# nuggy875/NeRF_pytorch_paeng

Hardware: AMD Instinct MI355X
Metric: rays/sec (4096-ray batch, 64c+128f samples) + 800×800 frame render ms (higher is better)
Workload: dtype f32

## Files before the change

### nerf_pytorch_paeng_amd/csrc/mlp_train.hip

```cpp
#include <type_traits>
#include <vector>
#include "mlp_core.h"
#include "half_layout.h"

namespace minerf {

int stage_embed(const float*, const float*, int64_t, int, int, int, float*, hipStream_t);
int dgrad_f16s(const mi_nerf_net*, const void*, const float*, const float*, const float*, const unsigned*, const unsigned*, float*, float*, float*, int64_t, int,
               long long, long long, const unsigned*, hipStream_t);

struct DgradArgs {
    const char* stream;
    unsigned stream_bytes;
    const float* side;
    unsigned side_floats, o_dens_w, o_color_w;
    const float* d_raw;
    const unsigned* mask_h;
    const unsigned* mask_g;
    float* delta_h;
    float* delta_f;
    float* delta_d;
    long long P;
    long long n_valid;
    long long n_wtiles;
    int S, tpr;
    int D;
};

template <int NT>
__device__ __forceinline__ void acc_zero(f32x16 (&acc)[8]) {
#pragma unroll
    for (int t = 0; t < NT; ++t)
#pragma unroll
        for (int r = 0; r < 16; ++r) acc[t][r] = 0.0f;
}

template <int W>
__global__ __launch_bounds__(256) __attribute__((amdgpu_waves_per_eu(1, 1)))
void mlp_dgrad_kernel(const DgradArgs a) {
    constexpr int NT = W / 32;
    constexpr int HN = W / 2;
    constexpr int AL = 8;
    extern __shared__ __attribute__((aligned(16))) char smem[];
    float* side = (float*)(smem + RING_BYTES);
    const int tid = threadIdx.x;
    const int lane = tid & 63;
    const int wave = __builtin_amdgcn_readfirstlane(tid >> 6);
    const int col = lane & 31, hh = lane >> 5;

    for (unsigned i = tid * 4; i < a.side_floats; i += 256 * 4) *(f32x4*)(side + i) = *(const f32x4*)(a.side + i);

    const long long n_wg_tiles = (a.n_wtiles + 3) >> 2;
    if ((long long)blockIdx.x >= n_wg_tiles) return;

    WRing ring = ring_start(a.stream, a.stream_bytes, smem, wave, lane);

    f32x16 acc[8];
    f32x4 aq[8];
    float h[HN];
    ring_advance(ring);
#pragma unroll
    for (int t = 0; t < NT; ++t) aq[t] = ring_read(smem, ring, lane, t);

    const float* cw = side + a.o_color_w;
    const float* dw = side + a.o_dens_w;
    for (long long wgt = blockIdx.x; wgt < n_wg_tiles; wgt += gridDim.x) {
        long long wt = wgt * 4 + wave;
        const bool wave_active = wt < a.n_wtiles;
        if (!wave_active) wt = a.n_wtiles - 1;
        const long long ray = wt / a.tpr;
        const int sample = (int)(wt - ray * a.tpr) * 32 + col;
        long long idx = ray * a.S + (sample < a.S ? sample : a.S - 1);
        const bool valid = wave_active && sample < a.S && idx < a.n_valid;
        if (idx >= a.n_valid) idx = a.n_valid - 1;
        const f32x4 dr = *(const f32x4*)(a.d_raw + idx * 4);
        const u32x2 mgv = *(const u32x2*)(a.mask_g + (wt * 64 + lane) * 2);
        u32x4 mhv = *(const u32x4*)(a.mask_h + (((long long)(a.D - 1) * a.n_wtiles + wt) * 64 + lane) * 4);

        float h2[HN / 2];
        {
            const unsigned mg[2] = {mgv[0], mgv[1]};
#pragma unroll
            for (int q = 0; q < HN / 8; ++q) {
                const f32x4 w0 = *(const f32x4*)(cw + 8 * q + 4 * hh);
                const f32x4 w1 = *(const f32x4*)(cw + W / 2 + 8 * q + 4 * hh);
                const f32x4 w2 = *(const f32x4*)(cw + W + 8 * q + 4 * hh);
#pragma unroll
                for (int e = 0; e < 4; ++e) {
                    float v = dr[0] * w0[e];
                    v = __builtin_fmaf(dr[1], w1[e], v);
                    v = __builtin_fmaf(dr[2], w2[e], v);
                    h2[4 * q + e] = mask_apply(v, q, e, mg);
                }
            }
        }
        acc_zero<NT>(acc);
        {
            float* row = a.delta_d + idx * (W / 2) + 4 * hh;
            auto hook = [&](int kq, int t) __attribute__((always_inline)) { if (t == NT - 1) store_chunk(h2, kq, row); };
            gemm_part<NT, HN / 2, NT, AL>(acc, h2, aq, smem, ring, lane, hook);
        }
        acc_to_b<NT, false>(acc, h);
        acc_zero<NT>(acc);
        {
            float* row = a.delta_f + idx * W + 4 * hh;
            auto hook = [&](int kq, int t) __attribute__((always_inline)) { if (t == NT - 1) store_chunk(h, kq, row); };
            gemm_part<NT, HN, NT, AL>(acc, h, aq, smem, ring, lane, hook);
        }
        {
            const unsigned mw[4] = {mhv[0], mhv[1], mhv[2], mhv[3]};
            if (a.D > 1) mhv = *(const u32x4*)(a.mask_h + (((long long)(a.D - 2) * a.n_wtiles + wt) * 64 + lane) * 4);
            const float ds = dr[3];
#pragma unroll
            for (int q = 0; q < 4 * NT; ++q) {
                const f32x4 wv = *(const f32x4*)(dw + 8 * q + 4 * hh);
#pragma unroll
                for (int e = 0; e < 4; ++e)
                    h[4 * q + e] = mask_apply(__builtin_fmaf(wv[e], ds, acc[q >> 2][4 * (q & 3) + e]), q, e, mw);
            }
        }
#pragma unroll 1
        for (int l = a.D - 1; l > 0; --l) {
            float* row = a.delta_h + ((long long)l * a.P + idx) * W + 4 * hh;
            acc_zero<NT>(acc);
            auto hook = [&](int kq, int t) __attribute__((always_inline)) { if (t == NT - 1) store_chunk(h, kq, row); };
            gemm_part<NT, HN, NT, AL>(acc, h, aq, smem, ring, lane, hook);
            const unsigned mw[4] = {mhv[0], mhv[1], mhv[2], mhv[3]};
            if (l > 1) mhv = *(const u32x4*)(a.mask_h + (((long long)(l - 2) * a.n_wtiles + wt) * 64 + lane) * 4);
#pragma unroll
            for (int q = 0; q < 4 * NT; ++q)
#pragma unroll
                for (int e = 0; e < 4; ++e) h[4 * q + e] = mask_apply(acc[q >> 2][4 * (q & 3) + e], q, e, mw);
        }
        store_rows<NT>(h, a.delta_h + idx * W + 4 * hh, valid);
    }
    asm volatile("s_waitcnt vmcnt(0)" ::: "memory");
    __syncthreads();
}

constexpr int WG_MAXB = 12;
struct WgradArgs {
    const float* dlt[WG_MAXB]; const float* x[WG_MAXB];
    int ldd[WG_MAXB], ldx[WG_MAXB], M[WG_MAXB], N[WG_MAXB];
    int want_bias[WG_MAXB];
    long long P;
    float* partial;
    float* bpartial;
    int slices;
};
struct ReduceBatch {
    float* out[WG_MAXB]; float* bias[WG_MAXB];
    int ldo[WG_MAXB], M[WG_MAXB], N[WG_MAXB];
};

typedef unsigned u32x4 __attribute__((ext_vector_type(4)));
__device__ __forceinline__ __amdgpu_buffer_rsrc_t wg_rsrc(const float* base, long long row0, long long ld, long long P, int rows) {
    long long left = P - row0;
    left = left < 0 ? 0 : (left > rows ? rows : left);
    return __builtin_amdgcn_make_buffer_rsrc((void*)(base + row0 * ld), 0, (int)(left * ld * 4), 0x00020000);
}
__global__ __launch_bounds__(256) __attribute__((amdgpu_waves_per_eu(1, 1)))
void wgrad_big_kernel(const WgradArgs a) {
    constexpr int U = 6;
    __shared__ f32x4 bshare[2][64];
    const int lane = threadIdx.x & 63;
    const int wave = __builtin_amdgcn_readfirstlane(threadIdx.x >> 6);
    const int i = lane & 31, kh = lane >> 5;
    const unsigned nwg = gridDim.x * gridDim.y, v = blockIdx.y * gridDim.x + blockIdx.x;
    const unsigned xcd = v & 7, slot = v >> 3;
    const unsigned full = nwg >> 3, rem = nwg & 7;
    const unsigned flat = xcd * full + (xcd < rem ? xcd : rem) + slot;
    const int b = (int)(flat / gridDim.x);
    const unsigned slice = flat - (unsigned)b * gridDim.x;
    const int wm = wave >> 1, wn = wave & 1;
    const int m0 = wm * 128, n0 = wn * 128;
    const bool aok = m0 + 4 * i < a.M[b], bok = n0 + 4 * i < a.N[b];
    const float* abase = a.dlt[b];
    const float* bbase = a.x[b];
    const long long ldd = a.ldd[b], ldx = a.ldx[b];
    const bool want_bias = a.want_bias[b] != 0;

    f32x16 acc[4][4];
#pragma unroll
    for (int tm = 0; tm < 4; ++tm)
#pragma unroll
        for (int tn = 0; tn < 4; ++tn)
#pragma unroll
            for (int r = 0; r < 16; ++r) acc[tm][tn][r] = 0.0f;
    f32x4 bsum = {0.f, 0.f, 0.f, 0.f};

    const long long slices = gridDim.x;
    unsigned voa[U], vob[U];
#pragma unroll
    for (int u = 0; u < U; ++u) {
        voa[u] = aok ? (unsigned)(((2 * u + kh) * ldd + m0 + 4 * i) * 4) : 0x80000000u;
        vob[u] = bok ? (unsigned)(((2 * u + kh) * ldx + n0 + 4 * i) * 4) : 0x80000000u;
    }
    long long req_group = slice;
    f32x4 ca[U], cb[U], na[U], nb[U], fa[U], fb[U];
    __amdgpu_buffer_rsrc_t ra, rb;
    auto open_group = [&]() __attribute__((always_inline)) {
        const long long row0 = req_group * (2 * U);
        ra = wg_rsrc(abase, row0, ldd, a.P, 2 * U);
        rb = wg_rsrc(bbase, row0, ldx, a.P, 2 * U);
        req_group += slices;
    };
    auto request = [&](int u, f32x4& A, f32x4& B) __attribute__((always_inline)) {
        A = __builtin_bit_cast(f32x4, __builtin_amdgcn_raw_buffer_load_b128(ra, voa[u], 0, 0));
        B = __builtin_bit_cast(f32x4, __builtin_amdgcn_raw_buffer_load_b128(rb, vob[u], 0, 0));
    };
    open_group();
#pragma unroll
    for (int u = 0; u < U; ++u) request(u, ca[u], cb[u]);
    open_group();
#pragma unroll
    for (int u = 0; u < U; ++u) request(u, na[u], nb[u]);
    auto step = [&](auto PAR, f32x4 (&A)[U], f32x4 (&B)[U], f32x4 (&FA)[U], f32x4 (&FB)[U]) __attribute__((always_inline)) {
        constexpr int par = decltype(PAR)::value;
        open_group();
#pragma unroll
        for (int u = 0; u < U; ++u) {
#pragma unroll
            for (int tm = 0; tm < 4; ++tm)
#pragma unroll
                for (int tn = 0; tn < 4; ++tn)
                    acc[tm][tn] = __builtin_amdgcn_mfma_f32_32x32x2f32(A[u][tm], B[u][tn], acc[tm][tn], 0, 0, 0);
            if ((u & 1) == par) bsum += A[u];
            request(u, FA[u], FB[u]);
            __builtin_amdgcn_sched_barrier(0);
        }
    };
    const long long all_groups = (a.P + 2 * U - 1) / (2 * U);
    const long long n_groups = (all_groups + slices - 1) / slices;
    auto loop = [&](auto PAR) __attribute__((always_inline)) {
        long long g = 0;
        do {
            step(PAR, ca, cb, fa, fb);
            step(PAR, na, nb, ca, cb);
            step(PAR, fa, fb, na, nb);
            g += 3;
        } while (g < n_groups);
    };
    if (!want_bias) loop(std::integral_constant<int, -1>{});
    else if (wn == 0) loop(std::integral_constant<int, 0>{});
    else loop(std::integral_constant<int, 1>{});
    const int lane_o = (int)__builtin_amdgcn_mbcnt_hi(~0u, __builtin_amdgcn_mbcnt_lo(~0u, 0u));
    const int i_o = lane_o & 31, kh_o = lane_o >> 5;
    float* out = a.partial + ((size_t)b * a.slices + slice) * (256 * 256);
#pragma unroll
    for (int tm = 0; tm < 4; ++tm)
#pragma unroll
        for (int r = 0; r < 16; ++r) {
            const int m = m0 + 4 * ((r & 3) + 8 * (r >> 2) + 4 * kh_o) + tm;
            f32x4 v;
#pragma unroll
            for (int tn = 0; tn < 4; ++tn) asm volatile("v_accvgpr_read_b32 %0, %1" : "=v"(v[tn]) : "a"(acc[tm][tn][r]));
            *(f32x4*)(out + (size_t)m * 256 + n0 + 4 * i_o) = v;
        }
    if (want_bias) {
        if (wn == 1) bshare[wm][lane_o] = bsum;
        __syncthreads();
        if (wn == 0) {
            bsum += bshare[wm][lane_o];
            f32x4 sv;
#pragma unroll
            for (int e = 0; e < 4; ++e) sv[e] = bsum[e] + __shfl_xor(bsum[e], 32, 64);
            if (kh_o == 0) *(f32x4*)(a.bpartial + ((size_t)b * a.slices + slice) * 256 + m0 + 4 * i_o) = sv;
        }
    }
}

typedef _Float16 f16x8 __attribute__((ext_vector_type(8)));
__global__ __launch_bounds__(256) void absmax_kernel(const float* __restrict__ x, long long n, unsigned* __restrict__ out_bits) {
    float m = 0.0f;
    const long long n4 = ((uintptr_t)x & 15) == 0 ? n >> 2 : 0;
    for (long long i = (long long)blockIdx.x * 256 + threadIdx.x; i < n4; i += (long long)gridDim.x * 256) {
        const f32x4 v = ((const f32x4*)x)[i];
        m = __builtin_fmaxf(__builtin_fmaxf(m, __builtin_fmaxf(__builtin_fabsf(v[0]), __builtin_fabsf(v[1]))), __builtin_fmaxf(__builtin_fabsf(v[2]), __builtin_fabsf(v[3])));
    }
    for (long long i = 4 * n4 + (long long)blockIdx.x * 256 + threadIdx.x; i < n; i += (long long)gridDim.x * 256) m = __builtin_fmaxf(m, __builtin_fabsf(x[i]));
#pragma unroll
    for (int o = 32; o > 0; o >>= 1) m = __builtin_fmaxf(m, __shfl_xor(m, o, 64));
    if ((threadIdx.x & 63) == 0 && m == m) atomicMax(out_bits, __float_as_uint(m));
}
static void launch_absmax(const float* x, long long n, unsigned* out_bits, hipStream_t st) {
    long long blocks = (n / 4 + 255) / 256;
    blocks = blocks < 1 ? 1 : (blocks > 4096 ? 4096 : blocks);
    hipLaunchKernelGGL(absmax_kernel, dim3((unsigned)blocks), dim3(256), 0, st, x, n, out_bits);
}
template <bool S>
__device__ __forceinline__ void split_pair(float v0, float v1, float s, unsigned& hi, unsigned& lo) {
    if constexpr (S) { v0 *= s; v1 *= s; }
    asm("v_cvt_pk_f16_f32 %0, %1, %2" : "=v"(hi) : "v"(v0), "v"(v1));
    asm("v_fma_mixlo_f16 %0, %1, -1.0, %2 op_sel_hi:[1,0,0]\n\tv_fma_mixhi_f16 %0, %1, -1.0, %3 op_sel:[1,0,0] op_sel_hi:[1,0,0]"
        : "=&v"(lo) : "v"(hi), "v"(v0), "v"(v1));
}
template <int BIAS>
__device__ __forceinline__ void wgrad_f16s_body(const WgradArgs& a, const unsigned* absmax_bits, f32x4 (*bshare)[64]) {
    const int lane = threadIdx.x & 63;
    const int wave = __builtin_amdgcn_readfirstlane(threadIdx.x >> 6);
    const int i = lane & 31, kh = lane >> 5;
    const unsigned nwg = gridDim.x * gridDim.y, v = blockIdx.y * gridDim.x + blockIdx.x;
    const unsigned xcd = v & 7, slot = v >> 3;
    const unsigned full = nwg >> 3, rem = nwg & 7;
    const unsigned flat = xcd * full + (xcd < rem ? xcd : rem) + slot;
    const int b = (int)(flat / gridDim.x);
    const unsigned slice = flat - (unsigned)b * gridDim.x;
    const int wm = wave >> 1, wn = wave & 1;
    const int m0 = wm * 128, n0 = wn * 128;
    const bool aok = m0 + 4 * i < a.M[b], bok = n0 + 4 * i < a.N[b];
    const float* abase = a.dlt[b];
    const float* bbase = a.x[b];
    const long long ldd = a.ldd[b], ldx = a.ldx[b];
    const unsigned mb = __builtin_amdgcn_readfirstlane((int)*absmax_bits);
    int e = (int)((mb >> 23) & 255u) - 127;
    if (mb == 0u || e < -100) e = -100;
    if (e > 100) e = 100;
    const float sc = __uint_as_float((unsigned)(127 + 7 - e) << 23), inv_sc = __uint_as_float((unsigned)(127 - 7 + e) << 23);

    f32x16 acc[4][4];
#pragma unroll
    for (int tm = 0; tm < 4; ++tm)
#pragma unroll
        for (int tn = 0; tn < 4; ++tn)
#pragma unroll
            for (int r = 0; r < 16; ++r) acc[tm][tn][r] = 0.0f;
    f32x4 bsum = {0.f, 0.f, 0.f, 0.f};

    constexpr int GROUP = 32;
    const long long slices = gridDim.x;
    unsigned voa[4], vob[4];
#pragma unroll
    for (int r = 0; r < 4; ++r) {
        voa[r] = aok ? (unsigned)(((8 * kh + r) * ldd + m0 + 4 * i) * 4) : 0x80000000u;
        vob[r] = bok ? (unsigned)(((8 * kh + r) * ldx + n0 + 4 * i) * 4) : 0x80000000u;
    }
    long long req_group = slice;
    struct Unit { f32x4 A[4], B[4]; };
    auto request = [&](int q, Unit& u) __attribute__((always_inline)) {
        const long long row0 = req_group * GROUP + 16 * (q >> 1) + 4 * (q & 1);
        const __amdgpu_buffer_rsrc_t ra = wg_rsrc(abase, row0, ldd, a.P, 12), rb = wg_rsrc(bbase, row0, ldx, a.P, 12);
#pragma unroll
        for (int r = 0; r < 4; ++r) {
            u.A[r] = __builtin_bit_cast(f32x4, __builtin_amdgcn_raw_buffer_load_b128(ra, voa[r], 0, 0));
            u.B[r] = __builtin_bit_cast(f32x4, __builtin_amdgcn_raw_buffer_load_b128(rb, vob[r], 0, 0));
        }
    };
    auto open_group = [&]() __attribute__((always_inline)) { req_group += slices; };
    unsigned ahi[4][4], alo[4][4], bhi[4][4], blo[4][4];
    auto convert = [&](int h, const Unit& u) __attribute__((always_inline)) {
#pragma unroll
        for (int t = 0; t < 4; ++t)
#pragma unroll
            for (int pr = 0; pr < 2; ++pr) {
                split_pair<true>(u.A[2 * pr][t], u.A[2 * pr + 1][t], sc, ahi[t][2 * h + pr], alo[t][2 * h + pr]);
                split_pair<false>(u.B[2 * pr][t], u.B[2 * pr + 1][t], 1.0f, bhi[t][2 * h + pr], blo[t][2 * h + pr]);
            }
        if constexpr (BIAS) {
#pragma unroll
            for (int r = 0; r < 4; ++r) bsum += u.A[r];
        }
    };
    auto mfmas = [&]() __attribute__((always_inline)) {
        f16x8 AH[4], AL[4], BH[4], BL[4];
#pragma unroll
        for (int t = 0; t < 4; ++t) {
            u32x4 w;
            w[0] = ahi[t][0]; w[1] = ahi[t][1]; w[2] = ahi[t][2]; w[3] = ahi[t][3]; AH[t] = __builtin_bit_cast(f16x8, w);
            w[0] = alo[t][0]; w[1] = alo[t][1]; w[2] = alo[t][2]; w[3] = alo[t][3]; AL[t] = __builtin_bit_cast(f16x8, w);
            w[0] = bhi[t][0]; w[1] = bhi[t][1]; w[2] = bhi[t][2]; w[3] = bhi[t][3]; BH[t] = __builtin_bit_cast(f16x8, w);
            w[0] = blo[t][0]; w[1] = blo[t][1]; w[2] = blo[t][2]; w[3] = blo[t][3]; BL[t] = __builtin_bit_cast(f16x8, w);
        }
#pragma unroll
        for (int tm = 0; tm < 4; ++tm)
#pragma unroll
            for (int tn = 0; tn < 4; ++tn) {
                acc[tm][tn] = __builtin_amdgcn_mfma_f32_32x32x16_f16(AH[tm], BH[tn], acc[tm][tn], 0, 0, 0);
                acc[tm][tn] = __builtin_amdgcn_mfma_f32_32x32x16_f16(AH[tm], BL[tn], acc[tm][tn], 0, 0, 0);
                acc[tm][tn] = __builtin_amdgcn_mfma_f32_32x32x16_f16(AL[tm], BH[tn], acc[tm][tn], 0, 0, 0);
            }
    };
    Unit u0, u1, u2, u3;
    request(0, u0); request(1, u1); request(2, u2); request(3, u3);
    const long long all_groups = (a.P + GROUP - 1) / GROUP;
    const long long n_groups = (all_groups + slices - 1) / slices;
    for (long long g = 0; g < n_groups; ++g) {
        open_group();
        convert(0, u0); request(0, u0);
        convert(1, u1); request(1, u1);
        mfmas();
        convert(0, u2); request(2, u2);
        convert(1, u3); request(3, u3);
        mfmas();
    }
    const int lane_o = (int)__builtin_amdgcn_mbcnt_hi(~0u, __builtin_amdgcn_mbcnt_lo(~0u, 0u));
    const int i_o = lane_o & 31, kh_o = lane_o >> 5;
    float* out = a.partial + ((size_t)b * a.slices + slice) * (256 * 256);
#pragma unroll
    for (int tm = 0; tm < 4; ++tm)
#pragma unroll
        for (int r = 0; r < 16; ++r) {
            const int m = m0 + 4 * ((r & 3) + 8 * (r >> 2) + 4 * kh_o) + tm;
            f32x4 vv;
#pragma unroll
            for (int tn = 0; tn < 4; ++tn) { float t; asm volatile("v_accvgpr_read_b32 %0, %1" : "=v"(t) : "a"(acc[tm][tn][r])); vv[tn] = t * inv_sc; }
            *(f32x4*)(out + (size_t)m * 256 + n0 + 4 * i_o) = vv;
        }
    if (a.want_bias[b] != 0) {
        if constexpr (BIAS) {
            f32x4 sv;
#pragma unroll
            for (int c = 0; c < 4; ++c) sv[c] = bsum[c] + __shfl_xor(bsum[c], 32, 64);
            if (kh_o == 0) *(f32x4*)(a.bpartial + ((size_t)b * a.slices + slice) * 256 + m0 + 4 * i_o) = sv;
        }
    }
    (void)bshare;
}
__global__ __launch_bounds__(256) __attribute__((amdgpu_waves_per_eu(1, 1)))
void wgrad_f16s_kernel(const WgradArgs a, const unsigned* absmax_bits) {
    asm volatile("s_setreg_imm32_b32 hwreg(HW_REG_MODE, 23, 1), 1");
    const int wave = __builtin_amdgcn_readfirstlane(threadIdx.x >> 6);
    if ((wave & 1) == 0) wgrad_f16s_body<1>(a, absmax_bits, nullptr);
    else wgrad_f16s_body<0>(a, absmax_bits, nullptr);
}

struct NarrowArgs {
    const float* wide; int ldw; int Mw;
    const float* nar;  int ldn; int Nn;
    long long P;
    int pps;
    float* partial;
    float* wsum;
    float* nsum;
};

template <int WQ, int NN, bool BW, bool BN>
__global__ __launch_bounds__(256) __attribute__((amdgpu_waves_per_eu(1, (WQ * NN == 4) ? 1 : 2)))
void wgrad_narrow_kernel(const NarrowArgs a) {
    constexpr int U = (WQ == 2) ? 4 : 6;
    const int lane = threadIdx.x & 63;
    const int wave = __builtin_amdgcn_readfirstlane(threadIdx.x >> 6);
    const int i = lane & 31, kh = lane >> 5;
    const long long slice = (long long)blockIdx.x * 4 + wave;
    const long long pb = slice * a.pps;
    const long long pe = pb >= a.P ? pb : ((pb + a.pps < a.P) ? pb + a.pps : a.P);
    const long long ldw = a.ldw, ldn = a.ldn;

    unsigned vow[U][WQ], von[U][NN];
#pragma unroll
    for (int u = 0; u < U; ++u) {
#pragma unroll
        for (int q = 0; q < WQ; ++q) vow[u][q] = (128 * q + 4 * i < a.Mw) ? (unsigned)(((2 * u + kh) * ldw + 128 * q + 4 * i) * 4) : 0x80000000u;
#pragma unroll
        for (int q = 0; q < NN; ++q) von[u][q] = (32 * q + i < a.Nn) ? (unsigned)(((2 * u + kh) * ldn + 32 * q + i) * 4) : 0x80000000u;
    }

    f32x16 acc[4 * WQ][NN];
#pragma unroll
    for (int tm = 0; tm < 4 * WQ; ++tm)
#pragma unroll
        for (int tn = 0; tn < NN; ++tn)
#pragma unroll
            for (int r = 0; r < 16; ++r) acc[tm][tn][r] = 0.0f;
    f32x4 wsum[WQ];
    float nsum[NN];
#pragma unroll
    for (int q = 0; q < WQ; ++q) wsum[q] = f32x4{0.f, 0.f, 0.f, 0.f};
#pragma unroll
    for (int q = 0; q < NN; ++q) nsum[q] = 0.0f;

    struct Set { f32x4 w[U][WQ]; float n[U][NN]; };
    Set c, nx, f;
    long long req_row = pb;
    __amdgpu_buffer_rsrc_t rw, rn;
    auto open_group = [&]() __attribute__((always_inline)) {
        rw = wg_rsrc(a.wide, req_row, ldw, pe, 2 * U);
        rn = wg_rsrc(a.nar, req_row, ldn, pe, 2 * U);
        req_row += 2 * U;
    };
    auto request = [&](Set& S, int u) __attribute__((always_inline)) {
#pragma unroll
        for (int q = 0; q < WQ; ++q) S.w[u][q] = __builtin_bit_cast(f32x4, __builtin_amdgcn_raw_buffer_load_b128(rw, vow[u][q], 0, 0));
#pragma unroll
        for (int q = 0; q < NN; ++q) S.n[u][q] = __builtin_bit_cast(float, __builtin_amdgcn_raw_buffer_load_b32(rn, von[u][q], 0, 0));
    };
    open_group();
#pragma unroll
    for (int u = 0; u < U; ++u) request(c, u);
    open_group();
#pragma unroll
    for (int u = 0; u < U; ++u) request(nx, u);
    auto step = [&](Set& A, Set& F) __attribute__((always_inline)) {
        open_group();
#pragma unroll
        for (int u = 0; u < U; ++u) {
#pragma unroll
            for (int tm = 0; tm < 4 * WQ; ++tm)
#pragma unroll
                for (int tn = 0; tn < NN; ++tn)
                    acc[tm][tn] = __builtin_amdgcn_mfma_f32_32x32x2f32(A.w[u][tm >> 2][tm & 3], A.n[u][tn], acc[tm][tn], 0, 0, 0);
            if (BW) {
#pragma unroll
                for (int q = 0; q < WQ; ++q) wsum[q] += A.w[u][q];
            }
            if (BN) {
#pragma unroll
                for (int q = 0; q < NN; ++q) nsum[q] += A.n[u][q];
            }
            request(F, u);
            __builtin_amdgcn_sched_barrier(0);
        }
    };
    const long long n_groups = (pe - pb + 2 * U - 1) / (2 * U);
    for (long long g = 0; g < n_groups; g += 3) {
        step(c, f);
        step(nx, c);
        step(f, nx);
    }
    constexpr int Wp = 128 * WQ, Np = 32 * NN;
    __shared__ float red[3][16][64];
    const __amdgpu_buffer_rsrc_t rout = __builtin_amdgcn_make_buffer_rsrc((void*)(a.partial + (size_t)blockIdx.x * Wp * Np), 0, Wp * Np * 4, 0x00020000);
    const unsigned vout = (unsigned)((16 * kh * Np + i) * 4);
#pragma unroll
    for (int tm = 0; tm < 4 * WQ; ++tm)
#pragma unroll
        for (int tn = 0; tn < NN; ++tn) {
            float t[16];
#pragma unroll
            for (int r = 0; r < 16; ++r) asm volatile("v_accvgpr_read_b32 %0, %1" : "=v"(t[r]) : "a"(acc[tm][tn][r]));
            if (wave > 0) {
#pragma unroll
                for (int r = 0; r < 16; ++r) red[wave - 1][r][lane] = t[r];
            }
            __syncthreads();
            if (wave == 0) {
#pragma unroll
                for (int r = 0; r < 16; ++r) {
                    const float v = ((t[r] + red[0][r][lane]) + red[1][r][lane]) + red[2][r][lane];
                    const int w0 = 128 * (tm >> 2) + 4 * ((r & 3) + 8 * (r >> 2)) + (tm & 3);
                    __builtin_amdgcn_raw_buffer_store_b32(__builtin_bit_cast(unsigned, v), rout, vout, (w0 * Np + 32 * tn) * 4, 0);
                }
            }
            __syncthreads();
        }
    float* sums = &red[0][0][0];
#pragma unroll
    for (int q = 0; q < WQ; ++q)
#pragma unroll
        for (int e = 0; e < 4; ++e) {
            const float v = wsum[q][e] + __shfl_xor(wsum[q][e], 32, 64);
            if (kh == 0) sums[wave * (Wp + Np) + 128 * q + 4 * i + e] = v;
        }
#pragma unroll
    for (int q = 0; q < NN; ++q) {
        const float v = nsum[q] + __shfl_xor(nsum[q], 32, 64);
        if (kh == 0) sums[wave * (Wp + Np) + Wp + 32 * q + i] = v;
    }
    __syncthreads();
    for (int c = threadIdx.x; c < Wp + Np; c += 256) {
        const float v = ((sums[c] + sums[(Wp + Np) + c]) + sums[2 * (Wp + Np) + c]) + sums[3 * (Wp + Np) + c];
        if (c < Wp) { if (a.wsum) a.wsum[(size_t)blockIdx.x * Wp + c] = v; }
        else if (a.nsum) a.nsum[(size_t)blockIdx.x * Np + (c - Wp)] = v;
    }
}

__global__ __launch_bounds__(256) void reduce_partial_kernel(const float* __restrict__ partial, const float* __restrict__ bpartial,
                                                              int slices, int Mp, int Np, int M, int N, float* __restrict__ out, int ldo,
                                                              float* __restrict__ bias, int bias_pitch, int transposed) {
    __shared__ float red[4][64];
    const int g = threadIdx.x >> 6, o = threadIdx.x & 63;
    const int idx = blockIdx.x * 64 + o;
    const int total = M * N + (bias ? M : 0);
    float acc = 0.0f;
    if (idx < M * N) {
        const int m = idx / N, n = idx - m * N;
        const float* p = partial + (transposed ? (size_t)n * Np + m : (size_t)m * Np + n);
        const size_t stride = (size_t)Mp * Np;
        float s[8] = {0.f, 0.f, 0.f, 0.f, 0.f, 0.f, 0.f, 0.f};
        int sl = g;
        for (; sl + 28 < slices; sl += 32) {
#pragma unroll
            for (int k = 0; k < 8; ++k) s[k] += p[(size_t)(sl + 4 * k) * stride];
        }
        for (; sl < slices; sl += 4) s[0] += p[(size_t)sl * stride];
        acc = ((s[0] + s[1]) + (s[2] + s[3])) + ((s[4] + s[5]) + (s[6] + s[7]));
    } else if (idx < total) {
        const int m = idx - M * N;
        for (int sl = g; sl < slices; sl += 4) acc += bpartial[(size_t)sl * bias_pitch + m];
    }
    red[g][o] = acc;
    __syncthreads();
    if (g == 0 && idx < total) {
        const float v = ((red[0][o] + red[1][o]) + red[2][o]) + red[3][o];
        if (idx < M * N) { const int m = idx / N, n = idx - m * N; out[(size_t)m * ldo + n] = v; }
        else bias[idx - M * N] = v;
    }
}

__global__ __launch_bounds__(256) void reduce_batch_kernel(const float* __restrict__ partial, const float* __restrict__ bpartial, int slices,
                                                            const ReduceBatch rb) {
    __shared__ float red[4][64];
    const int b = blockIdx.y;
    const int M = rb.M[b], N = rb.N[b];
    const int g = threadIdx.x >> 6, o = threadIdx.x & 63;
    const int idx = blockIdx.x * 64 + o;
    const int total = M * N + (rb.bias[b] ? M : 0);
    float acc = 0.0f;
    if (idx < M * N) {
        const int m = idx / N, n = idx - m * N;
        const float* p = partial + (size_t)b * slices * 65536 + (size_t)m * 256 + n;
        float s[8] = {0.f, 0.f, 0.f, 0.f, 0.f, 0.f, 0.f, 0.f};
        int sl = g;
        for (; sl + 28 < slices; sl += 32) {
#pragma unroll
            for (int k = 0; k < 8; ++k) s[k] += p[(size_t)(sl + 4 * k) * 65536];
        }
        for (; sl < slices; sl += 4) s[0] += p[(size_t)sl * 65536];
        acc = ((s[0] + s[1]) + (s[2] + s[3])) + ((s[4] + s[5]) + (s[6] + s[7]));
    } else if (idx < total) {
        const int m = idx - M * N;
        for (int sl = g; sl < slices; sl += 4) acc += bpartial[((size_t)b * slices + sl) * 256 + m];
    }
    red[g][o] = acc;
    __syncthreads();
    if (g == 0 && idx < total) {
        const float v = ((red[0][o] + red[1][o]) + red[2][o]) + red[3][o];
        if (idx < M * N) { const int m = idx / N, n = idx - m * N; rb.out[b][(size_t)m * rb.ldo[b] + n] = v; }
        else rb.bias[b][idx - M * N] = v;
    }
}

__global__ __launch_bounds__(256) void pack_apply_kernel(const int32_t* __restrict__ map, const float* __restrict__ flat, long long n,
                                                          float* __restrict__ blob) {
    const long long i = (long long)blockIdx.x * 256 + threadIdx.x;
    if (i >= n) return;
    const int32_t m = map[i];
    blob[i] = m > 0 ? flat[m - 1] : 0.0f;
}


static inline size_t al256(size_t v) { return (v + 255) & ~(size_t)255; }
constexpr size_t WGRAD_OVERRUN_PAD = 128 * 1024;

constexpr size_t WGRAD_PARTIAL_FLOATS = (size_t)256 * 256 * 256 + (size_t)256 * 256;

int train_layout(const mi_nerf_net* net, int64_t n_rays, int S, mi_nerf_train_layout* L) {
    MN_CHECK_ARG(net && L, "NULL net/layout");
    MN_CHECK_ARG(native_width(net->W), "the training kernels exist for W = 128 and 256 (got %d; inference pads narrower networks)", net->W);
    MN_CHECK_ARG(net->D >= 2 && net->D <= 16, "unsupported depth D=%d", net->D);
    MN_CHECK_ARG(n_rays >= 0 && S >= 1, "bad sizes n_rays=%lld S=%d", (long long)n_rays, S);
    const size_t p = (size_t)n_rays * S, W = (size_t)net->W, D = (size_t)net->D;
    const size_t n_wtiles = (size_t)n_rays * ((S + 31) / 32);
    const size_t in_all = (size_t)(3 + 6 * net->L_x) + (size_t)(3 + 6 * net->L_d);
    size_t off = 0;
    L->stash_h = off; off += al256(D * p * W * 4);
    L->stash_f = off; off += al256(p * W * 4);
    L->stash_g = off; off += al256(p * (W / 2) * 4) + WGRAD_OVERRUN_PAD;
    L->mask_h = off;  off += al256(D * n_wtiles * 64 * 16);
    L->mask_g = off;  off += al256(n_wtiles * 64 * 8);
    L->stash_bytes = off;
    off = 0;
    L->delta_h = off; off += al256(D * p * W * 4);
    L->delta_f = off; off += al256(p * W * 4);
    L->delta_d = off; off += al256(p * (W / 2) * 4) + WGRAD_OVERRUN_PAD;
    L->emb = off;     off += al256(p * in_all * 4);
    L->partial = off; off += al256(WGRAD_PARTIAL_FLOATS * 4);
    off += 256;
    L->work_bytes = off;
    return MI_NERF_OK;
}

struct WideProduct { const float* dlt; int ldd, M; const float* x; int ldx, N; float* out; int ldo; float* bias; };

static int run_wgrad_batch(const WideProduct* pr, int n, long long P, float* partial, hipStream_t st, const unsigned* absmax = nullptr) {
    MN_CHECK_ARG(n >= 1 && n <= WG_MAXB, "%d wide products in one batch (at most WG_MAXB)", n);
    WgradArgs a{};
    ReduceBatch rb{};
    int max_total = 0;
    for (int b = 0; b < n; ++b) {
        const WideProduct& q = pr[b];
        MN_CHECK_ARG(q.M <= 256 && q.N <= 256 && q.M % 4 == 0 && q.N % 4 == 0 && q.ldd % 4 == 0 && q.ldx % 4 == 0 &&
                     ((uintptr_t)q.dlt & 15) == 0 && ((uintptr_t)q.x & 15) == 0,
                     "wgrad operands must be at most 256 wide, 16-byte aligned, with pitches of 4 floats");
        a.dlt[b] = q.dlt; a.x[b] = q.x; a.ldd[b] = q.ldd; a.ldx[b] = q.ldx; a.M[b] = q.M; a.N[b] = q.N; a.want_bias[b] = q.bias != nullptr;
        rb.out[b] = q.out; rb.bias[b] = q.bias; rb.ldo[b] = q.ldo; rb.M[b] = q.M; rb.N[b] = q.N;
        const int total = q.M * q.N + (q.bias ? q.M : 0);
        if (total > max_total) max_total = total;
    }
    int slices = device_cus() / n;
    const long long all_groups = (P + 11) / 12;
    if (slices > all_groups) slices = (int)all_groups;
    if (slices < 1) slices = 1;
    MN_CHECK_ARG((size_t)n * slices * (65536 + 256) <= WGRAD_PARTIAL_FLOATS, "internal: wgrad partial buffer too small");
    a.P = P; a.slices = slices;
    a.partial = partial;
    a.bpartial = partial + (size_t)n * slices * 65536;
    if (absmax) hipLaunchKernelGGL(wgrad_f16s_kernel, dim3(slices, n), dim3(256), 0, st, a, absmax);
    else hipLaunchKernelGGL(wgrad_big_kernel, dim3(slices, n), dim3(256), 0, st, a);
    MN_LAUNCH_CHECK("wgrad_big_kernel");
    hipLaunchKernelGGL(reduce_batch_kernel, dim3((max_total + 63) / 64, n), dim3(256), 0, st, (const float*)partial, (const float*)a.bpartial,
                       slices, rb);
    MN_LAUNCH_CHECK("reduce_batch_kernel");
    return MI_NERF_OK;
}

static int run_wgrad(const float* dlt, int ldd, int M, const float* x, int ldx, int N, long long P, float* out, int ldo, float* bias,
                     float* partial, hipStream_t st) {
    if (M > 64 && N > 64) {
        const WideProduct q{dlt, ldd, M, x, ldx, N, out, ldo, bias};
        return run_wgrad_batch(&q, 1, P, partial, st);
    }
    const bool delta_is_wide = M >= N;
    NarrowArgs a{};
    a.wide = delta_is_wide ? dlt : x; a.ldw = delta_is_wide ? ldd : ldx; a.Mw = delta_is_wide ? M : N;
    a.nar = delta_is_wide ? x : dlt;  a.ldn = delta_is_wide ? ldx : ldd; a.Nn = delta_is_wide ? N : M;
    a.P = P;
    MN_CHECK_ARG(a.Mw <= 256 && a.Nn <= 64 && a.Mw % 4 == 0 && a.ldw % 4 == 0 && ((uintptr_t)a.wide & 15) == 0,
                 "unsupported narrow wgrad shape %d x %d", M, N);
    const int WQ = a.Mw > 128 ? 2 : 1, NN = a.Nn > 32 ? 2 : 1;
    const int Wp = 128 * WQ, Np = 32 * NN;
    const size_t per_slice = (size_t)Wp * Np + Wp + Np;
    long long wslices = 4LL * device_cus();
    long long pps = (P + wslices - 1) / wslices;
    pps = (pps + 23) / 24 * 24;
    wslices = (P + pps - 1) / pps;
    const long long slices = (wslices + 3) / 4;
    MN_CHECK_ARG((size_t)slices * per_slice <= WGRAD_PARTIAL_FLOATS, "internal: wgrad partial buffer too small");
    a.pps = (int)pps;
    a.partial = partial;
    float* wsum = partial + (size_t)slices * Wp * Np;
    float* nsum = wsum + (size_t)slices * Wp;
    a.wsum = (bias && delta_is_wide) ? wsum : nullptr;
    a.nsum = (bias && !delta_is_wide) ? nsum : nullptr;
    const dim3 grid((unsigned)slices);
    const bool bw = a.wsum != nullptr, bn = a.nsum != nullptr;
#define MN_NARROW(WQ_, NN_)                                                                                                   \
    do {                                                                                                                      \
        if (bw) hipLaunchKernelGGL((wgrad_narrow_kernel<WQ_, NN_, true, false>), grid, dim3(256), 0, st, a);                  \
        else if (bn) hipLaunchKernelGGL((wgrad_narrow_kernel<WQ_, NN_, false, true>), grid, dim3(256), 0, st, a);             \
        else hipLaunchKernelGGL((wgrad_narrow_kernel<WQ_, NN_, false, false>), grid, dim3(256), 0, st, a);                    \
    } while (0)
    if (WQ == 2 && NN == 2) MN_NARROW(2, 2);
    else if (WQ == 2) MN_NARROW(2, 1);
    else if (NN == 2) MN_NARROW(1, 2);
    else MN_NARROW(1, 1);
#undef MN_NARROW
    MN_LAUNCH_CHECK("wgrad_narrow_kernel");
    const int total = M * N + (bias ? M : 0);
    hipLaunchKernelGGL(reduce_partial_kernel, dim3((total + 63) / 64), dim3(256), 0, st, (const float*)partial,
                       (const float*)(delta_is_wide ? wsum : nsum), (int)slices, Wp, Np, M, N, out, ldo, bias, delta_is_wide ? Wp : Np,
                       delta_is_wide ? 0 : 1);
    MN_LAUNCH_CHECK("reduce_partial_kernel");
    return MI_NERF_OK;
}

size_t wgrad_scratch_bytes() { return WGRAD_PARTIAL_FLOATS * 4 + 256; }

int wgrad_products(int n, const float* const* dlt, const int* ldd, const int* M, const float* const* x, const int* ldx, const int* N, int64_t P,
                   float* const* out, const int* ldo, float* const* bias, void* scratch, size_t scratch_bytes, hipStream_t st, bool f16s) {
    MN_CHECK_ARG(n >= 1 && n <= WG_MAXB, "between 1 and %d products per launch (got %d)", WG_MAXB, n);
    MN_CHECK_ARG(P >= 1 && dlt && ldd && M && x && ldx && N && out && ldo && scratch, "bad sizes / NULL pointer");
    MN_CHECK_ARG(scratch_bytes >= wgrad_scratch_bytes(), "scratch too small: %zu < %zu", scratch_bytes, wgrad_scratch_bytes());
    WideProduct pr[WG_MAXB];
    int n_wide = 0;
    for (int b = 0; b < n; ++b) {
        MN_CHECK_ARG(dlt[b] && x[b] && out[b] && M[b] >= 1 && N[b] >= 1 && ldd[b] >= M[b] && ldx[b] >= N[b] && ldo[b] >= N[b],
                     "product %d: bad sizes M=%d N=%d (pitches %d / %d / %d) or NULL pointer", b, M[b], N[b], ldd[b], ldx[b], ldo[b]);
        const bool wide = M[b] > 64 && N[b] > 64;
        MN_CHECK_ARG(wide || !f16s, "product %d: the split-precision entry takes wide products (more than 64 columns on both sides), M=%d N=%d", b, M[b], N[b]);
        if (wide) pr[n_wide++] = WideProduct{dlt[b], ldd[b], M[b], x[b], ldx[b], N[b], out[b], ldo[b], bias ? bias[b] : nullptr};
    }
    unsigned* absmax = nullptr;
    if (f16s) {
        absmax = (unsigned*)((char*)scratch + WGRAD_PARTIAL_FLOATS * 4);
        MN_HIP(hipMemsetAsync(absmax, 0, 4, st));
        for (int b = 0; b < n; ++b) {
            MN_CHECK_ARG(ldd[b] == M[b], "product %d: the split-precision entry takes gradient operands without row padding (ldd == M)", b);
            launch_absmax(dlt[b], (long long)P * M[b], absmax, st);
        }
        MN_LAUNCH_CHECK("absmax_kernel");
    }
    if (n_wide)
        if (int rc = run_wgrad_batch(pr, n_wide, P, (float*)scratch, st, absmax)) return rc;
    for (int b = 0; b < n; ++b)
        if (!(M[b] > 64 && N[b] > 64))
            if (int rc = run_wgrad(dlt[b], ldd[b], M[b], x[b], ldx[b], N[b], P, out[b], ldo[b], bias ? bias[b] : nullptr, (float*)scratch, st)) return rc;
    return MI_NERF_OK;
}

template <int W>
static int launch_dgrad(const DgradArgs& a, hipStream_t st) {
    const size_t lds = RING_BYTES + (size_t)a.side_floats * 4;
    MN_CHECK_ARG(lds <= 160 * 1024, "LDS budget exceeded: %zu bytes", lds);
    auto kern = mlp_dgrad_kernel<W>;
    static LdsOptIn opt_in = {};
    if (int rc = ensure_lds_opt_in(opt_in, (const void*)kern)) return rc;
    const long long n_wg = (a.n_wtiles + 3) / 4;
    const int grid = persistent_grid(n_wg);
    hipLaunchKernelGGL(kern, dim3(grid), dim3(256), lds, st, a);
    MN_LAUNCH_CHECK("mlp_dgrad_kernel");
    return MI_NERF_OK;
}

int mlp_backward_fp32(const mi_nerf_net* net, const void* packed_fwd, const void* packed_bwd, const float* rays, const float* z,
                      int64_t n_rays, int S, const float* d_raw, const void* stash, void* work, size_t work_bytes, float* grads,
                      int stage, hipStream_t st, const float* x_dev, int64_t n_rows, int mode) {
    MN_CHECK_ARG(net != nullptr, "net is NULL");
    MN_CHECK_ARG(net->L_x >= 0 && net->L_x <= KERNEL_LX && net->L_d >= 0 && net->L_d <= KERNEL_LD, "unsupported encoding L_x=%d L_d=%d", net->L_x, net->L_d);
    MN_CHECK_ARG(net->skip >= -1, "bad skip=%d", net->skip);
    MN_CHECK_ARG(n_rays >= 0 && S >= 1, "bad sizes n_rays=%lld S=%d", (long long)n_rays, S);
    const long long Ppad = (long long)n_rays * S;
    const long long P = x_dev ? n_rows : Ppad;
    MN_CHECK_ARG(!x_dev || (S == 32 && n_rows >= 0 && n_rays == (n_rows + 31) / 32), "embedded mode wants (n_rays, S) = (ceil(n / 32), 32)");
    mi_nerf_train_layout L;
    if (int rc = train_layout(net, n_rays, S, &L)) return rc;
    if (P == 0) {
        if (grads && stage != 1) {
            MN_CHECK_ARG(net->D >= 1 && net->D <= 16 && (net->W == 128 || net->W == 256), "unsupported network D=%d W=%d", net->D, net->W);
            MN_HIP(hipMemsetAsync(grads, 0, (size_t)make_param_offsets(net->D, net->W, net->skip, net->L_x, net->L_d).total * 4, st));
        }
        if ((mode & 3) && work && work_bytes >= L.work_bytes)
            MN_HIP(hipMemsetAsync((char*)work + L.partial + al256(WGRAD_PARTIAL_FLOATS * 4), 0, 8, st));
        return MI_NERF_OK;
    }
    MN_CHECK_ARG(packed_fwd && packed_bwd && (x_dev || (rays && z)) && d_raw && stash && work && grads, "NULL device pointer");
    MN_CHECK_ARG(work_bytes >= L.work_bytes, "workspace too small: %zu < %zu", work_bytes, L.work_bytes);
    const int D = net->D, W = net->W;
    const int in_x = 3 + 6 * net->L_x, in_d = 3 + 6 * net->L_d, in_all = in_x + in_d;
    const BlobLayout BL = make_layout(D, W, net->skip, net->L_x, net->L_d);
    const ParamOffsets po = make_param_offsets(D, W, net->skip, net->L_x, net->L_d);
    const float* stash_h = (const float*)((const char*)stash + L.stash_h);
    const float* stash_f = (const float*)((const char*)stash + L.stash_f);
    const float* stash_g = (const float*)((const char*)stash + L.stash_g);
    float* delta_h = (float*)((char*)work + L.delta_h);
    float* delta_f = (float*)((char*)work + L.delta_f);
    float* delta_d = (float*)((char*)work + L.delta_d);
    float* emb = (float*)((char*)work + L.emb);
    float* partial = (float*)((char*)work + L.partial);

    DgradArgs a{};
    a.stream = (const char*)packed_bwd + HEADER_BYTES;
    a.stream_bytes = bwd_stream_bytes(D, W);
    a.side = (const float*)((const char*)packed_fwd + BL.side_off);
    a.side_floats = BL.side_floats; a.o_dens_w = BL.dens_w; a.o_color_w = BL.color_w;
    a.d_raw = d_raw;
    a.mask_h = (const unsigned*)((const char*)stash + L.mask_h);
    a.mask_g = (const unsigned*)((const char*)stash + L.mask_g);
    a.delta_h = delta_h; a.delta_f = delta_f; a.delta_d = delta_d;
    a.S = S; a.tpr = (S + 31) / 32;
    a.P = Ppad; a.n_valid = P; a.n_wtiles = (long long)n_rays * a.tpr; a.D = D;
    unsigned* absmax = nullptr;
    if (mode & 3) {
        MN_CHECK_ARG(!(mode & 2) || D <= F16S_DGRAD_MAX_D, "the split-precision backward-data kernel keeps a tile's ReLU' words of all layers in LDS: "
                     "D = %d does not fit (D <= %d); the fp32 backward-data kernel reads the same stash", D, F16S_DGRAD_MAX_D);
        MN_CHECK_ARG(W == 256 && !x_dev, "the split-precision backward is built for W=256 and the ray entry point");
        absmax = (unsigned*)((char*)work + L.partial + al256(WGRAD_PARTIAL_FLOATS * 4));
        MN_HIP(hipMemsetAsync(absmax, 0, 8, st));
        launch_absmax(d_raw, (long long)P * 4, absmax, st);
        MN_LAUNCH_CHECK("absmax_kernel");
    }
    if (mode & 2) {
        if (int rc = dgrad_f16s(net, packed_bwd, a.side + a.o_color_w, a.side + a.o_dens_w, d_raw, a.mask_h, a.mask_g, delta_h, delta_f, delta_d, n_rays, S,
                                Ppad, P, absmax, st)) return rc;
    } else {
        if (int rc = (W == 256 ? launch_dgrad<256>(a, st) : launch_dgrad<128>(a, st))) return rc;
    }
    if (stage == 1) return MI_NERF_OK;

    const float* embc = x_dev;
    if (!x_dev) {
        if (int rc = stage_embed(rays, z, n_rays, S, net->L_x, net->L_d, emb, st)) return rc;
        embc = emb;
    }
    const size_t PW = (size_t)Ppad * W;
    if (!(mode & 1)) absmax = nullptr;
    const float* h_last = stash_h + (size_t)(D - 1) * PW;
    {
        WideProduct pr[WG_MAXB];
        int n = 0;
        auto flush = [&]() -> int {
            const int rc = n ? run_wgrad_batch(pr, n, P, partial, st, absmax) : MI_NERF_OK;
            n = 0;
            return rc;
        };
        for (int l = 1; l < D; ++l) {
            const bool cat = po.in_l[l] != W;
            pr[n++] = WideProduct{delta_h + (size_t)l * PW, W, W, stash_h + (size_t)(l - 1) * PW, W, W, grads + po.w_x[l] + (cat ? in_x : 0),
                                  po.in_l[l], grads + po.b_x[l]};
            if (n == WG_MAXB) if (int rc = flush()) return rc;
        }
        pr[n++] = WideProduct{delta_f, W, W, h_last, W, W, grads + po.w_feat, W, grads + po.b_feat};
        if (n == WG_MAXB) if (int rc = flush()) return rc;
        pr[n++] = WideProduct{delta_d, W / 2, W / 2, stash_f, W, W, grads + po.w_d, W + in_d, grads + po.b_d};
        if (int rc = flush()) return rc;
    }
    if (int rc = run_wgrad(delta_h, W, W, embc, in_all, in_x, P, grads + po.w_x[0], in_x, grads + po.b_x[0], partial, st)) return rc;
    for (int l = 1; l < D; ++l)
        if (po.in_l[l] != W)
            if (int rc = run_wgrad(delta_h + (size_t)l * PW, W, W, embc, in_all, in_x, P, grads + po.w_x[l], po.in_l[l], nullptr, partial, st)) return rc;
    if (int rc = run_wgrad(d_raw + 3, 4, 1, h_last, W, W, P, grads + po.w_dens, W, grads + po.b_dens, partial, st)) return rc;
    if (int rc = run_wgrad(delta_d, W / 2, W / 2, embc + in_x, in_all, in_d, P, grads + po.w_d + W, W + in_d, nullptr, partial, st)) return rc;
    if (int rc = run_wgrad(d_raw, 4, 3, stash_g, W / 2, W / 2, P, grads + po.w_color, W / 2, grads + po.b_color, partial, st)) return rc;
    return MI_NERF_OK;
}

int pack_apply(const int32_t* map_dev, const float* flat_dev, size_t blob_bytes, void* blob_dev, hipStream_t st) {
    MN_CHECK_ARG(map_dev && flat_dev && blob_dev, "NULL device pointer");
    MN_CHECK_ARG(blob_bytes % 4 == 0, "blob size must be a multiple of 4");
    const long long n = (long long)(blob_bytes / 4);
    if (n == 0) return MI_NERF_OK;
    hipLaunchKernelGGL(pack_apply_kernel, dim3((unsigned)((n + 255) / 256)), dim3(256), 0, st, map_dev, flat_dev, n, (float*)blob_dev);
    MN_LAUNCH_CHECK("pack_apply_kernel");
    return MI_NERF_OK;
}

}
```

Baseline: 491,100.

## Plan wgrad workgroups per product, packing two slices for narrow-M products

Measured after the change: 488,900. No clear change (-0.4%).

```diff
diff --git a/nerf_pytorch_paeng_amd/csrc/mlp_train.hip b/nerf_pytorch_paeng_amd/csrc/mlp_train.hip
--- a/nerf_pytorch_paeng_amd/csrc/mlp_train.hip
+++ b/nerf_pytorch_paeng_amd/csrc/mlp_train.hip
@@ -2,6 +2,7 @@
 #include <vector>
 #include "mlp_core.h"
 #include "half_layout.h"
+#include "wgrad_plan.h"
 
 namespace minerf {
 
@@ -138,15 +139,14 @@
     __syncthreads();
 }
 
-constexpr int WG_MAXB = 12;
+constexpr int WG_MAXB = WGRAD_MAXB;
 struct WgradArgs {
     const float* dlt[WG_MAXB]; const float* x[WG_MAXB];
     int ldd[WG_MAXB], ldx[WG_MAXB], M[WG_MAXB], N[WG_MAXB];
     int want_bias[WG_MAXB];
     long long P;
     float* partial;
-    float* bpartial;
-    int slices;
+    WgradPlan plan;
 };
 struct ReduceBatch {
     float* out[WG_MAXB]; float* bias[WG_MAXB];
@@ -166,14 +166,16 @@
     const int lane = threadIdx.x & 63;
     const int wave = __builtin_amdgcn_readfirstlane(threadIdx.x >> 6);
     const int i = lane & 31, kh = lane >> 5;
-    const unsigned nwg = gridDim.x * gridDim.y, v = blockIdx.y * gridDim.x + blockIdx.x;
+    const unsigned nwg = gridDim.x, v = blockIdx.x;
     const unsigned xcd = v & 7, slot = v >> 3;
     const unsigned full = nwg >> 3, rem = nwg & 7;
     const unsigned flat = xcd * full + (xcd < rem ? xcd : rem) + slot;
-    const int b = (int)(flat / gridDim.x);
-    const unsigned slice = flat - (unsigned)b * gridDim.x;
     const int wm = wave >> 1, wn = wave & 1;
-    const int m0 = wm * 128, n0 = wn * 128;
+    const WgradSpot spot = wgrad_spot(a.plan, (int)flat, wm);
+    const int b = spot.b;
+    const unsigned slice = (unsigned)spot.slice;
+    const bool has_slice = spot.slice < a.plan.S;
+    const int m0 = spot.m0, n0 = wn * 128;
     const bool aok = m0 + 4 * i < a.M[b], bok = n0 + 4 * i < a.N[b];
     const float* abase = a.dlt[b];
     const float* bbase = a.x[b];
@@ -189,7 +191,7 @@
             for (int r = 0; r < 16; ++r) acc[tm][tn][r] = 0.0f;
     f32x4 bsum = {0.f, 0.f, 0.f, 0.f};
 
-    const long long slices = gridDim.x;
+    const long long slices = a.plan.S;
     unsigned voa[U], vob[U];
 #pragma unroll
     for (int u = 0; u < U; ++u) {
@@ -209,12 +211,6 @@
         A = __builtin_bit_cast(f32x4, __builtin_amdgcn_raw_buffer_load_b128(ra, voa[u], 0, 0));
         B = __builtin_bit_cast(f32x4, __builtin_amdgcn_raw_buffer_load_b128(rb, vob[u], 0, 0));
     };
-    open_group();
-#pragma unroll
-    for (int u = 0; u < U; ++u) request(u, ca[u], cb[u]);
-    open_group();
-#pragma unroll
-    for (int u = 0; u < U; ++u) request(u, na[u], nb[u]);
     auto step = [&](auto PAR, f32x4 (&A)[U], f32x4 (&B)[U], f32x4 (&FA)[U], f32x4 (&FB)[U]) __attribute__((always_inline)) {
         constexpr int par = decltype(PAR)::value;
         open_group();
@@ -241,31 +237,40 @@
             g += 3;
         } while (g < n_groups);
     };
-    if (!want_bias) loop(std::integral_constant<int, -1>{});
-    else if (wn == 0) loop(std::integral_constant<int, 0>{});
-    else loop(std::integral_constant<int, 1>{});
-    const int lane_o = (int)__builtin_amdgcn_mbcnt_hi(~0u, __builtin_amdgcn_mbcnt_lo(~0u, 0u));
-    const int i_o = lane_o & 31, kh_o = lane_o >> 5;
-    float* out = a.partial + ((size_t)b * a.slices + slice) * (256 * 256);
-#pragma unroll
-    for (int tm = 0; tm < 4; ++tm)
-#pragma unroll
-        for (int r = 0; r < 16; ++r) {
-            const int m = m0 + 4 * ((r & 3) + 8 * (r >> 2) + 4 * kh_o) + tm;
-            f32x4 v;
-#pragma unroll
-            for (int tn = 0; tn < 4; ++tn) asm volatile("v_accvgpr_read_b32 %0, %1" : "=v"(v[tn]) : "a"(acc[tm][tn][r]));
-            *(f32x4*)(out + (size_t)m * 256 + n0 + 4 * i_o) = v;
-        }
+    if (has_slice) {
+        open_group();
+#pragma unroll
+        for (int u = 0; u < U; ++u) request(u, ca[u], cb[u]);
+        open_group();
+#pragma unroll
+        for (int u = 0; u < U; ++u) request(u, na[u], nb[u]);
+        if (!want_bias) loop(std::integral_constant<int, -1>{});
+        else if (wn == 0) loop(std::integral_constant<int, 0>{});
+        else loop(std::integral_constant<int, 1>{});
+        const int lane_o = (int)__builtin_amdgcn_mbcnt_hi(~0u, __builtin_amdgcn_mbcnt_lo(~0u, 0u));
+        const int i_o = lane_o & 31, kh_o = lane_o >> 5;
+        float* out = a.partial + a.plan.part_off[b] + (size_t)slice * a.plan.rows[b] * 256;
+#pragma unroll
+        for (int tm = 0; tm < 4; ++tm)
+#pragma unroll
+            for (int r = 0; r < 16; ++r) {
+                const int m = m0 + 4 * ((r & 3) + 8 * (r >> 2) + 4 * kh_o) + tm;
+                f32x4 v;
+#pragma unroll
+                for (int tn = 0; tn < 4; ++tn) asm volatile("v_accvgpr_read_b32 %0, %1" : "=v"(v[tn]) : "a"(acc[tm][tn][r]));
+                *(f32x4*)(out + (size_t)m * 256 + n0 + 4 * i_o) = v;
+            }
+    }
     if (want_bias) {
-        if (wn == 1) bshare[wm][lane_o] = bsum;
+        const int lane_o = (int)__builtin_amdgcn_mbcnt_hi(~0u, __builtin_amdgcn_mbcnt_lo(~0u, 0u));
+        if (wn == 1 && has_slice) bshare[wm][lane_o] = bsum;
         __syncthreads();
-        if (wn == 0) {
+        if (wn == 0 && has_slice) {
             bsum += bshare[wm][lane_o];
             f32x4 sv;
 #pragma unroll
             for (int e = 0; e < 4; ++e) sv[e] = bsum[e] + __shfl_xor(bsum[e], 32, 64);
-            if (kh_o == 0) *(f32x4*)(a.bpartial + ((size_t)b * a.slices + slice) * 256 + m0 + 4 * i_o) = sv;
+            if ((lane_o >> 5) == 0) *(f32x4*)(a.partial + a.plan.bias_off[b] + (size_t)slice * 256 + m0 + 4 * (lane_o & 31)) = sv;
         }
     }
 }
@@ -300,14 +305,15 @@
     const int lane = threadIdx.x & 63;
     const int wave = __builtin_amdgcn_readfirstlane(threadIdx.x >> 6);
     const int i = lane & 31, kh = lane >> 5;
-    const unsigned nwg = gridDim.x * gridDim.y, v = blockIdx.y * gridDim.x + blockIdx.x;
+    const unsigned nwg = gridDim.x, v = blockIdx.x;
     const unsigned xcd = v & 7, slot = v >> 3;
     const unsigned full = nwg >> 3, rem = nwg & 7;
     const unsigned flat = xcd * full + (xcd < rem ? xcd : rem) + slot;
-    const int b = (int)(flat / gridDim.x);
-    const unsigned slice = flat - (unsigned)b * gridDim.x;
     const int wm = wave >> 1, wn = wave & 1;
-    const int m0 = wm * 128, n0 = wn * 128;
+    const WgradSpot spot = wgrad_spot(a.plan, (int)flat, wm);
+    const int b = spot.b;
+    const unsigned slice = (unsigned)spot.slice;
+    const int m0 = spot.m0, n0 = wn * 128;
     const bool aok = m0 + 4 * i < a.M[b], bok = n0 + 4 * i < a.N[b];
     const float* abase = a.dlt[b];
     const float* bbase = a.x[b];
@@ -328,7 +334,7 @@
     f32x4 bsum = {0.f, 0.f, 0.f, 0.f};
 
     constexpr int GROUP = 32;
-    const long long slices = gridDim.x;
+    const long long slices = a.plan.S;
     unsigned voa[4], vob[4];
 #pragma unroll
     for (int r = 0; r < 4; ++r) {
@@ -395,7 +401,7 @@
     }
     const int lane_o = (int)__builtin_amdgcn_mbcnt_hi(~0u, __builtin_amdgcn_mbcnt_lo(~0u, 0u));
     const int i_o = lane_o & 31, kh_o = lane_o >> 5;
-    float* out = a.partial + ((size_t)b * a.slices + slice) * (256 * 256);
+    float* out = a.partial + a.plan.part_off[b] + (size_t)slice * a.plan.rows[b] * 256;
 #pragma unroll
     for (int tm = 0; tm < 4; ++tm)
 #pragma unroll
@@ -411,7 +417,7 @@
             f32x4 sv;
 #pragma unroll
             for (int c = 0; c < 4; ++c) sv[c] = bsum[c] + __shfl_xor(bsum[c], 32, 64);
-            if (kh_o == 0) *(f32x4*)(a.bpartial + ((size_t)b * a.slices + slice) * 256 + m0 + 4 * i_o) = sv;
+            if (kh_o == 0) *(f32x4*)(a.partial + a.plan.bias_off[b] + (size_t)slice * 256 + m0 + 4 * i_o) = sv;
         }
     }
     (void)bshare;
@@ -597,29 +603,30 @@
     }
 }
 
-__global__ __launch_bounds__(256) void reduce_batch_kernel(const float* __restrict__ partial, const float* __restrict__ bpartial, int slices,
-                                                            const ReduceBatch rb) {
+__global__ __launch_bounds__(256) void reduce_batch_kernel(const float* __restrict__ partial, const WgradPlan plan, const ReduceBatch rb) {
     __shared__ float red[4][64];
     const int b = blockIdx.y;
-    const int M = rb.M[b], N = rb.N[b];
+    const int M = rb.M[b], N = rb.N[b], slices = plan.S;
     const int g = threadIdx.x >> 6, o = threadIdx.x & 63;
     const int idx = blockIdx.x * 64 + o;
     const int total = M * N + (rb.bias[b] ? M : 0);
     float acc = 0.0f;
     if (idx < M * N) {
         const int m = idx / N, n = idx - m * N;
-        const float* p = partial + (size_t)b * slices * 65536 + (size_t)m * 256 + n;
+        const float* p = partial + plan.part_off[b] + (size_t)m * 256 + n;
+        const size_t stride = (size_t)plan.rows[b] * 256;
         float s[8] = {0.f, 0.f, 0.f, 0.f, 0.f, 0.f, 0.f, 0.f};
         int sl = g;
         for (; sl + 28 < slices; sl += 32) {
 #pragma unroll
-            for (int k = 0; k < 8; ++k) s[k] += p[(size_t)(sl + 4 * k) * 65536];
-        }
-        for (; sl < slices; sl += 4) s[0] += p[(size_t)sl * 65536];
+            for (int k = 0; k < 8; ++k) s[k] += p[(size_t)(sl + 4 * k) * stride];
+        }
+        for (; sl < slices; sl += 4) s[0] += p[(size_t)sl * stride];
         acc = ((s[0] + s[1]) + (s[2] + s[3])) + ((s[4] + s[5]) + (s[6] + s[7]));
     } else if (idx < total) {
         const int m = idx - M * N;
-        for (int sl = g; sl < slices; sl += 4) acc += bpartial[((size_t)b * slices + sl) * 256 + m];
+        const float* bp = partial + plan.bias_off[b];
+        for (int sl = g; sl < slices; sl += 4) acc += bp[(size_t)sl * 256 + m];
     }
     red[g][o] = acc;
     __syncthreads();
@@ -687,19 +694,14 @@
         const int total = q.M * q.N + (q.bias ? q.M : 0);
         if (total > max_total) max_total = total;
     }
-    int slices = device_cus() / n;
-    const long long all_groups = (P + 11) / 12;
-    if (slices > all_groups) slices = (int)all_groups;
-    if (slices < 1) slices = 1;
-    MN_CHECK_ARG((size_t)n * slices * (65536 + 256) <= WGRAD_PARTIAL_FLOATS, "internal: wgrad partial buffer too small");
-    a.P = P; a.slices = slices;
+    MN_CHECK_ARG(wgrad_plan(a.M, n, device_cus(), P, (long long)WGRAD_PARTIAL_FLOATS, absmax == nullptr, a.plan),
+                 "internal: wgrad partial buffer too small");
+    a.P = P;
     a.partial = partial;
-    a.bpartial = partial + (size_t)n * slices * 65536;
-    if (absmax) hipLaunchKernelGGL(wgrad_f16s_kernel, dim3(slices, n), dim3(256), 0, st, a, absmax);
-    else hipLaunchKernelGGL(wgrad_big_kernel, dim3(slices, n), dim3(256), 0, st, a);
+    if (absmax) hipLaunchKernelGGL(wgrad_f16s_kernel, dim3(a.plan.n_wg), dim3(256), 0, st, a, absmax);
+    else hipLaunchKernelGGL(wgrad_big_kernel, dim3(a.plan.n_wg), dim3(256), 0, st, a);
     MN_LAUNCH_CHECK("wgrad_big_kernel");
-    hipLaunchKernelGGL(reduce_batch_kernel, dim3((max_total + 63) / 64, n), dim3(256), 0, st, (const float*)partial, (const float*)a.bpartial,
-                       slices, rb);
+    hipLaunchKernelGGL(reduce_batch_kernel, dim3((max_total + 63) / 64, n), dim3(256), 0, st, (const float*)partial, a.plan, rb);
     MN_LAUNCH_CHECK("reduce_batch_kernel");
     return MI_NERF_OK;
 }
diff --git a/nerf_pytorch_paeng_amd/csrc/wgrad_plan.h b/nerf_pytorch_paeng_amd/csrc/wgrad_plan.h
--- /dev/null
+++ b/nerf_pytorch_paeng_amd/csrc/wgrad_plan.h
@@ -0,0 +1,82 @@
+#pragma once
+
+namespace minerf {
+
+constexpr int WGRAD_MAXB = 12;
+constexpr int WGRAD_GROUP_POINTS = 12;
+constexpr int WGRAD_MAX_SLICES = 256;
+
+struct WgradPlan {
+    int n;
+    int S;
+    int n_wg;
+    int wg0[WGRAD_MAXB];
+    int rows[WGRAD_MAXB];
+    long long part_off[WGRAD_MAXB];
+    long long bias_off[WGRAD_MAXB];
+    long long floats;
+};
+
+inline int wgrad_halves(int M) { return M <= 128 ? 1 : 2; }
+
+inline int wgrad_product_wgs(int M, int S, bool split_halves) {
+    return split_halves && wgrad_halves(M) == 1 ? (S + 1) / 2 : S;
+}
+
+inline void wgrad_plan_fill(WgradPlan& p, const int* M, int n, int S, bool split_halves) {
+    p.n = n;
+    p.S = S;
+    int wg = 0;
+    long long off = 0;
+    for (int b = 0; b < WGRAD_MAXB; ++b) {
+        p.wg0[b] = wg;
+        p.rows[b] = 256;
+        p.part_off[b] = off;
+        if (b >= n) continue;
+        p.rows[b] = split_halves && wgrad_halves(M[b]) == 1 ? 128 : 256;
+        wg += wgrad_product_wgs(M[b], S, split_halves);
+        off += (long long)S * p.rows[b] * 256;
+    }
+    p.n_wg = wg;
+    for (int b = 0; b < WGRAD_MAXB; ++b) {
+        p.bias_off[b] = off;
+        if (b < n) off += (long long)S * 256;
+    }
+    p.floats = off;
+}
+
+inline bool wgrad_plan(const int* M, int n, int cus, long long P, long long capacity, bool split_halves, WgradPlan& p) {
+    const long long all_groups = (P + WGRAD_GROUP_POINTS - 1) / WGRAD_GROUP_POINTS;
+    int S;
+    if (!split_halves) {
+        S = cus / n;
+        if (S > WGRAD_MAX_SLICES) S = WGRAD_MAX_SLICES;
+        if (S > all_groups) S = (int)all_groups;
+        if (S < 1) S = 1;
+        wgrad_plan_fill(p, M, n, S, false);
+        return p.floats <= capacity;
+    }
+    S = all_groups < WGRAD_MAX_SLICES ? (int)all_groups : WGRAD_MAX_SLICES;
+    if (S < 1) S = 1;
+    for (; S > 1; --S) {
+        wgrad_plan_fill(p, M, n, S, true);
+        if (p.n_wg <= cus && p.floats <= capacity) return true;
+    }
+    wgrad_plan_fill(p, M, n, 1, true);
+    return p.floats <= capacity;
+}
+
+struct WgradSpot {
+    int b;
+    int slice;
+    int m0;
+};
+constexpr WgradSpot wgrad_spot(const WgradPlan& p, int flat, int wm) {
+    int b = 0;
+    for (int k = 1; k < WGRAD_MAXB; ++k) b += flat >= p.wg0[k];
+    const int w = flat - p.wg0[b];
+    if (p.rows[b] == 128) return WgradSpot{b, 2 * w + wm, 0};
+    return WgradSpot{b, w, 128 * wm};
+}
+
+}
```
